# PoloWlg/Joint-Multimodal-Transformer-6th-ABAW

Hardware: AMD Instinct MI355X
Metric: train windows/sec + CCC parity, B=64 T=300 A/V fusion, 1/2/4/8 MI355X (higher is better)
Workload: dtype bf16; 1 GPU; configs[2]: FcLayer(1024,512) + Two_transformers(TRANSFORMER,FC,H=1,L=1,vision_in_ft=2048) + 2x CCCLoss + SGD-nesterov; global_batch=64, per_gpu_batch=64, seq_len=300, D_a=1024, D_v=2048, parallelism=dp1

## Files before the change

### include/jmt.h

```cpp
#ifndef JMT_H_
#define JMT_H_

#include <stddef.h>
#include <stdint.h>

#ifdef __cplusplus
extern "C" {
#endif

#define JMT_ABI_VERSION 7

enum { JMT_F32 = 0, JMT_BF16 = 1, JMT_F16 = 2 };
enum { JMT_OK = 0, JMT_ERR_ARG = -1, JMT_ERR_HIP = -2, JMT_ERR_UNSUPPORTED = -3 };

int jmt_abi_version(void);
const char* jmt_last_error(void);
int jmt_kernel_count(void);
long long jmt_bounds_violations(int reset);

typedef struct jmt_gemm_desc {
  int ab_dtype, c_dtype, aux_dtype;
  int M, N, K;
  const void* a[8];
  const void* b[8];
  void* c[8];
  int n_a, n_b, n_c;
  int a_mode, b_mode, c_mode;
  int a_kseg, b_kseg;
  int a_kmajor, b_kmajor;
  int64_t lda, ldb, ldc, ldaux;
  int batch0, batch1;
  int64_t sA0, sA1, sB0, sB1, sC0, sC1;
  float alpha, beta;
  const float* bias;
  int bias_mode;
  int relu;
  const void* aux;
  int splits;
  void* workspace;
  size_t ws_bytes;
  const float* bias_tab[8];
  int n_bias;
  float* dbias_tab[8];
  int n_dbias;
  int dbias_acc;
  float* dbias_ws;
  size_t dbias_ws_bytes;
} jmt_gemm_desc;

int jmt_gemm(const jmt_gemm_desc* desc, void* stream);
int jmt_gemm_cin(const jmt_gemm_desc* desc, const void* const* c_in, int n_c_in, int64_t ldcin,
                 void* stream);
int jmt_gemm_persist_cfg(const jmt_gemm_desc* desc);
size_t jmt_gemm_workspace_bytes(int M, int N, int batch, int splits);
int jmt_gemm_plan_splits(int ab_dtype, int M, int N, int K, int batch);
void jmt_gemm_set_debug(int flags);
int jmt_gemm_trace_read(uint64_t* host, int nblocks);

int jmt_gemm_grouped(const jmt_gemm_desc* descs, int n, void* workspace, size_t ws_bytes,
                     void* stream);
size_t jmt_gemm_grouped_workspace_bytes(const jmt_gemm_desc* descs, int n);
int jmt_gemm_grouped_plan(const jmt_gemm_desc* descs, int n, int* splits_out);

int jmt_gemm_group16(const jmt_gemm_desc* descs, int n, void* stream);
int jmt_gemm_group16_ok(const jmt_gemm_desc* descs, int n);
void jmt_gemm_group16_set_grid(int blocks);


int jmt_l2norm_fwd(int x_dt, int y_dt, int64_t rows, int D, const void* x, int64_t ldx, void* y,
                   int64_t ldy, float* inv_norm, float eps, void* stream);
int jmt_l2norm_bwd(int x_dt, int dy_dt, int dx_dt, int64_t rows, int D, const void* x,
                   int64_t ldx, const void* dy, int64_t lddy, const float* inv_norm, float eps,
                   void* dx, int64_t lddx, void* stream);

int jmt_layernorm_fwd(int dt_in, int dt_out, int64_t rows, int D, const void* x, int64_t ldx,
                      const void* r, int64_t ldr, const float* gamma, const float* beta, float eps,
                      void* y, int64_t ldy, float* mean, float* rstd, void* stream);
int jmt_layernorm_bwd_blocks(int64_t rows);
int jmt_layernorm_bwd(int dt_in, int dt_dy, int dt_dx, int64_t rows, int D, const void* x,
                      int64_t ldx, const void* r, int64_t ldr, const void* dy, int64_t lddy,
                      const float* mean, const float* rstd, const float* gamma, void* dx,
                      int64_t lddx, float* dgamma, float* dbeta, int beta_acc, float* partials,
                      void* stream);

int jmt_layernorm_bwd_dsum(int dt_in, int dt_dy, int dt_dx, int64_t rows, int D, const void* x,
                           int64_t ldx, const void* r, int64_t ldr, const void* dy, int64_t lddy,
                           const float* mean, const float* rstd, const float* gamma, void* dx,
                           int64_t lddx, float* dgamma, float* dbeta, float* dsum, int beta_acc,
                           float* partials, void* stream);

int jmt_layernorm_fwd_grouped(int dt_in, int dt_out, int G, int64_t rows, int D, const void* x,
                              int64_t ldx, int64_t sx, const void* r, int64_t ldr, int64_t sr,
                              const float* const* gamma, const float* const* beta, float eps,
                              void* y, int64_t ldy, int64_t sy, float* mean, float* rstd,
                              void* stream);
int jmt_layernorm_bwd_grouped(int dt_in, int dt_dy, int dt_dx, int G, int64_t rows, int D,
                              const void* x, int64_t ldx, int64_t sx, const void* r, int64_t ldr,
                              int64_t sr, const void* dy, int64_t lddy, int64_t sdy,
                              const float* mean, const float* rstd, const float* const* gamma,
                              void* dx, int64_t lddx, int64_t sdx, float* const* dgamma,
                              float* const* dbeta, float* const* dsum, int beta_acc,
                              float* partials, void* stream);
int jmt_layernorm_bwd_grouped_blocks(int64_t rows);

int jmt_softmax_fwd(int p_dt, int64_t rows, int n, const float* s, int64_t lds, float scale,
                    void* p, int64_t ldp, void* stream);
int jmt_softmax_bwd(int p_dt, int ds_dt, int64_t rows, int n, const void* p, int64_t ldp,
                    const float* dp, int64_t lddp, float scale, void* ds, int64_t ldds,
// ... 294 lines not shown
```

### joint-multimodal-transformer-6th-abaw_amd/csrc/gemm.hip

```cpp
#include "gemm_tile.h"

namespace jmt {

struct GemmWork {
  int m0, n0, b, b0, b1, split, kbeg, kend;
};

template <class C>
__device__ __forceinline__ GemmWork decode_work(const GemmParams& p, int w) {
  const int ntile = p.tiles_m * p.tiles_n;
  const int nb = p.batch0 * p.batch1;
  const bool global = p.splits > 1 && !(p.dbg & 16);
  if (global) {
    const int W = ntile * nb * p.splits;
    const int q = W / 8, rm = W % 8, x = w % 8;
    w = x * q + min(x, rm) + w / 8;
  }
  const int bid = w % ntile;
  const int rest = w / ntile;
  GemmWork r;
  r.b = rest % nb;
  r.split = rest / nb;
  int wg = bid;
  if (!global && ntile >= 16) {
// ... 515 lines not shown
      cfg = 44;
      splits = s;
      return;
    }
  }
  const TileModel* ms = dt == JMT_F32 ? kModels32 : kModels16;
  const int nm = dt == JMT_F32 ? 1 : 2;
  double best = 1e300;
  cfg = 1;
  splits = fixed_splits > 0 ? fixed_splits : 1;
  for (int i = 0; i < nm; ++i) {
    if (!tile_ok(ms[i], M, N)) continue;
    const long tiles = (long)((M + ms[i].bm - 1) / ms[i].bm) * ((N + ms[i].bn - 1) / ms[i].bn) *
                       batch;
    int s_lo = 1, s_hi = tiles <= 8 ? 256 : 32;
    if (fixed_splits > 0) s_lo = s_hi = fixed_splits;
    for (int s = s_lo; s <= s_hi; ++s) {
      if (fixed_splits <= 0 && s > 1 && K / s < 4 * bke) break;
      const double c = model_cost(ms[i], M, N, K, batch, s, bke);
      if (c < best * 0.999) { best = c; cfg = ms[i].id; splits = s; }
    }
  }
}

}

using namespace jmt;

static int g_gemm_dbg = 0;
static int g_gemm_cfg = 0;
extern "C" int jmt_gemm_trace_read(uint64_t* host, int nblocks) {
  if (nblocks > kTraceBlocks) nblocks = kTraceBlocks;
  if (hipDeviceSynchronize() != hipSuccess ||
      hipMemcpyFromSymbol(host, HIP_SYMBOL(g_gemm_trace), sizeof(uint64_t) * 4 * nblocks) !=
          hipSuccess)
    return -1;
  return nblocks;
}
extern "C" void jmt_gemm_set_debug(int flags) { g_gemm_dbg = flags & 0xff; g_gemm_cfg = flags >> 8; }

extern "C" int jmt_gemm_plan_splits(int ab_dtype, int M, int N, int K, int batch) {
  if (M <= 0 || N <= 0 || K <= 0) return 1;
  if (ab_dtype != JMT_F32 && ab_dtype != JMT_BF16 && ab_dtype != JMT_F16) return 1;
  int cfg, splits;
  plan(ab_dtype, M, N, K, batch < 1 ? 1 : batch, 0, cfg, splits);
  return splits;
}

extern "C" size_t jmt_gemm_workspace_bytes(int M, int N, int batch, int splits) {
  if (splits <= 1) return 0;
  return (size_t)splits * (size_t)batch * (size_t)M * (size_t)N * sizeof(float);
}

static int gemm_run(const jmt_gemm_desc* d, bool cin, const void* const* c_in, int n_c_in,
                    int64_t ldcin, void* stream, int* plan_out = nullptr) {
  JMT_CHECK_ARG(d != nullptr, "jmt_gemm: null descriptor");
  const int dt = d->ab_dtype;
  JMT_CHECK_ARG(dt == JMT_F32 || dt == JMT_BF16 || dt == JMT_F16, "jmt_gemm: bad ab_dtype %d", dt);
  JMT_CHECK_ARG(d->c_dtype == JMT_F32 || d->c_dtype == dt, "jmt_gemm: c_dtype must be f32 or ab");
  JMT_CHECK_ARG(d->M >= 0 && d->N >= 0 && d->K >= 0, "jmt_gemm: negative size");
  JMT_CHECK_ARG(d->aux == nullptr || d->aux_dtype == d->c_dtype,
                "jmt_gemm: aux (ReLU mask) must have the output dtype");
  if (d->M == 0 || d->N == 0) return JMT_OK;
  const int batch0 = d->batch0 < 1 ? 1 : d->batch0;
  const int batch1 = d->batch1 < 1 ? 1 : d->batch1;
  JMT_CHECK_ARG(batch0 * batch1 <= 65535, "jmt_gemm: batch too large");
  const int es = dtype_size(dt);
  const int V = 16 / es;
  const int BKE = 128 / es;
  JMT_CHECK_ARG(d->n_a >= 1 && d->n_a <= MAXP && d->n_b >= 1 && d->n_b <= MAXP &&
                    d->n_c >= 1 && d->n_c <= MAXP, "jmt_gemm: pointer table size");
  JMT_CHECK_ARG(d->lda % V == 0 && d->ldb % V == 0, "jmt_gemm: lda/ldb must be multiples of %d", V);
  JMT_CHECK_ARG((d->sA0 % V == 0) && (d->sA1 % V == 0) && (d->sB0 % V == 0) && (d->sB1 % V == 0),
                "jmt_gemm: batch strides must be multiples of %d elements", V);
  for (int i = 0; i < d->n_a; ++i)
    JMT_CHECK_ARG(((uintptr_t)d->a[i] & 15) == 0, "jmt_gemm: A[%d] not 16-B aligned", i);
  for (int i = 0; i < d->n_b; ++i)
    JMT_CHECK_ARG(((uintptr_t)d->b[i] & 15) == 0, "jmt_gemm: B[%d] not 16-B aligned", i);
  JMT_CHECK_ARG(d->a_mode >= 0 && d->a_mode <= 3 && d->b_mode >= 0 && d->b_mode <= 3 &&
                    d->c_mode >= 0 && d->c_mode <= 1, "jmt_gemm: bad operand mode");
  if (d->a_mode == 2) JMT_CHECK_ARG(d->a_kseg % BKE == 0 && d->a_kseg * d->n_a >= d->K,
                                    "jmt_gemm: A K-concat segment must be a multiple of %d", BKE);
  if (d->b_mode == 2) JMT_CHECK_ARG(d->b_kseg % BKE == 0 && d->b_kseg * d->n_b >= d->K,
                                    "jmt_gemm: B K-concat segment must be a multiple of %d", BKE);
  const int nseg_a = d->a_mode == 3 && d->a_kseg > 0 ? (d->K + d->a_kseg - 1) / d->a_kseg : 1;
  const int nseg_b = d->b_mode == 3 && d->b_kseg > 0 ? (d->K + d->b_kseg - 1) / d->b_kseg : 1;
  if (d->a_mode == 3) JMT_CHECK_ARG(d->a_kseg > 0 && d->a_kseg % BKE == 0 &&
                                        d->n_a >= batch0 * nseg_a && d->batch1 <= 1,
                                    "jmt_gemm: A per-batch K-concat needs kseg a multiple of %d, "
                                    "batch0 x ceil(K / kseg) pointers and batch1 = 1", BKE);
  if (d->b_mode == 3) JMT_CHECK_ARG(d->b_kseg > 0 && d->b_kseg % BKE == 0 &&
                                        d->n_b >= batch0 * nseg_b && d->batch1 <= 1,
                                    "jmt_gemm: B per-batch K-concat needs kseg a multiple of %d, "
                                    "batch0 x ceil(K / kseg) pointers and batch1 = 1", BKE);
  if (d->a_mode == 1) JMT_CHECK_ARG(d->n_a >= batch0, "jmt_gemm: A pointer table < batch0");
  if (d->b_mode == 1) JMT_CHECK_ARG(d->n_b >= batch0, "jmt_gemm: B pointer table < batch0");
  if (d->c_mode == 1) JMT_CHECK_ARG(d->n_c >= batch0, "jmt_gemm: C pointer table < batch0");

  GemmParams p;
  for (int i = 0; i < MAXP; ++i) {
    p.a_ptr[i] = i < d->n_a ? d->a[i] : nullptr;
    p.b_ptr[i] = i < d->n_b ? d->b[i] : nullptr;
    p.c_ptr[i] = i < d->n_c ? d->c[i] : nullptr;
  }
  JMT_CHECK_ARG(d->n_bias >= 0 && d->n_bias <= MAXP, "jmt_gemm: bias table size");
  if (d->n_bias > 0)
    JMT_CHECK_ARG(d->n_bias >= batch0 && d->bias_mode != 0, "jmt_gemm: bias table < batch0");
  p.bias = d->bias;
// ... 27 lines not shown
                  "dbias table of batch0 entries");
    bool any = false;
    for (int i = 0; i < batch0; ++i) any = any || d->dbias_tab[i] != nullptr;
    JMT_CHECK_ARG(any, "jmt_gemm: every dbias_tab entry is null");
  }
  {
    const int ces = dtype_size(d->c_dtype);
    bool cv4 = d->ldc % 4 == 0 && d->sC0 % 4 == 0 && d->sC1 % 4 == 0;
    for (int i = 0; i < d->n_c; ++i) cv4 = cv4 && (((uintptr_t)d->c[i] & (4 * ces - 1)) == 0);
    if (d->aux) cv4 = cv4 && (((uintptr_t)d->aux & (4 * ces - 1)) == 0) && d->ldaux % 4 == 0;
    p.c_vec4 = cv4 ? 1 : 0;
    bool cv8 = cv4 && d->ldc % 8 == 0 && d->sC0 % 8 == 0 && d->sC1 % 8 == 0;
    for (int i = 0; i < d->n_c; ++i) cv8 = cv8 && (((uintptr_t)d->c[i] & 15) == 0);
    p.c_vec8 = cv8 ? 1 : 0;
  }

  for (int i = 0; i < MAXP; ++i) p.cin_ptr[i] = p.c_ptr[i];
  p.ldcin = d->ldc;
  if (cin) {
    JMT_CHECK_ARG(d->beta != 0.f, "jmt_gemm_cin: beta == 0 reads no C operand");
    JMT_CHECK_ARG(c_in != nullptr && n_c_in >= (d->c_mode == 1 ? batch0 : 1) && n_c_in <= MAXP,
                  "jmt_gemm_cin: c_in table null or shorter than C's");
    for (int i = 0; i < n_c_in; ++i)
      JMT_CHECK_ARG(c_in[i] != nullptr && ((uintptr_t)c_in[i] & 15) == 0,
                    "jmt_gemm_cin: c_in[%d] null or not 16-B aligned", i);
    JMT_CHECK_ARG(ldcin >= d->N && ldcin % 8 == 0,
                  "jmt_gemm_cin: ldcin must be a multiple of 8 elements, at least N");
    if (d->c_dtype == JMT_F32 || dt == JMT_F32)
      return set_error(JMT_ERR_UNSUPPORTED, "jmt_gemm_cin: 16-bit C only");
    if (d->splits > 1)
      return set_error(JMT_ERR_UNSUPPORTED, "jmt_gemm_cin: split-K reduces into C itself");
    for (int i = 0; i < MAXP; ++i) p.cin_ptr[i] = i < n_c_in ? c_in[i] : nullptr;
    p.ldcin = ldcin;
  }

  int splits = d->splits < 1 ? 1 : d->splits;
  int kps = ((d->K + splits - 1) / splits + BKE - 1) / BKE * BKE;
  if (kps < BKE) kps = BKE;
  splits = (d->K + kps - 1) / kps;
  if (splits < 1) splits = 1;
  p.splits = splits;
  p.k_per_split = splits > 1 ? kps : (d->K > 0 ? d->K : 1);
  p.ws = (float*)d->workspace;
  if (splits > 1) {
    const size_t need = jmt_gemm_workspace_bytes(d->M, d->N, batch0 * batch1, splits);
    JMT_CHECK_ARG(d->workspace != nullptr && d->ws_bytes >= need,
                  "jmt_gemm: split-K needs %zu workspace bytes", need);
    if (d->n_dbias > 0) {
      const size_t dneed = (size_t)splits * batch0 * (size_t)d->M * sizeof(float);
      JMT_CHECK_ARG(d->dbias_ws != nullptr && d->dbias_ws_bytes >= dneed,
                    "jmt_gemm: split-K A row sums need %zu dbias_ws bytes", dneed);
    }
  }
  int cfg = g_gemm_cfg;
  {
    const int pc = persist_choice(d, p, splits, cfg);
    if (plan_out) {
      *plan_out = pc;
      return JMT_OK;
    }
    if (pc) {
      p.tiles_m = (d->M + 255) / 256;
      p.tiles_n = d->N / 256;
      const int W = p.tiles_m * p.tiles_n * batch0 * batch1;
      const int ncu = num_cus_persist();
      const int blocks = W < ncu ? W : ncu;
      launch_gemm_persist(p, dt, d->a_kmajor, d->b_kmajor, pc, blocks, as_stream(stream));
      JMT_LAUNCH_CHECK("jmt_gemm(persistent)");
      return JMT_OK;
    }
  }
  const bool pp_split = splits > 1 && pp_split_ok(dt, d->M, d->N, d->K, splits) &&
                        (cfg == 44 || (cfg == 0 && pp_split_env() &&
                                       pp_split_plan(dt, d->M, d->N, d->K, batch0 * batch1)));
  if (cfg == 44) cfg = 0;
  if (cfg == 40 || cfg == 43 || cfg == 45) cfg = 5;
  if (dt == JMT_F32 && cfg >= 10) cfg = 1;
  if (cfg == 32 && !d->a_kmajor) cfg = 5;
  if (!cfg) {
    int s_unused;
    plan(dt, d->M, d->N, d->K, batch0 * batch1, splits, cfg, s_unused);
    if (dt != JMT_F32 && (cfg == 1 || splits == 1)) {
      const int t = occupancy_override(d->a_kmajor, d->b_kmajor, d->M, d->N, d->K,
                                       batch0 * batch1, splits);
      if (t) cfg = t;
    }
  }
  if (d->n_dbias > 0 && cfg == 10) cfg = 5;
  hipStream_t st = as_stream(stream);
  if (pp_split) {
    p.tiles_m = d->M / 256;
    p.tiles_n = d->N / 256;
    const int W = p.tiles_m * p.tiles_n * batch0 * batch1 * splits;
    const int ncu = num_cus_persist();
    launch_gemm_pp_split(p, dt, d->a_kmajor, d->b_kmajor, d->n_dbias > 0, W < ncu ? W : ncu, st);
    JMT_LAUNCH_CHECK("jmt_gemm(split-K ping-pong)");
  } else {
    int bm, bn;
    cfg_tile(cfg, bm, bn);
    p.tiles_m = (d->M + bm - 1) / bm;
    p.tiles_n = (d->N + bn - 1) / bn;
    dim3 grid(p.tiles_m * p.tiles_n, batch0 * batch1, splits);
    if (dt == JMT_F32) launch_t<float>(p, d->a_kmajor, d->b_kmajor, cfg, grid, st);
    else if (dt == JMT_BF16) launch_t<__bf16>(p, d->a_kmajor, d->b_kmajor, cfg, grid, st);
    else launch_t<_Float16>(p, d->a_kmajor, d->b_kmajor, cfg, grid, st);
    JMT_LAUNCH_CHECK("jmt_gemm");
  }
  if (splits > 1) {
    const bool v4 = d->N % 4 == 0 && p.c_vec4;
    const int64_t total = (int64_t)d->M * d->N * batch0 * batch1 / (v4 ? 4 : 1);
    int blocks = (int)((total + 255) / 256);
    if (blocks > 8192) blocks = 8192;
#define JMT_SKR(O)                                                                          \
    if (v4) hipLaunchKernelGGL((splitk_reduce_kernel<O, true>), dim3(blocks), dim3(256), 0, st, p); \
    else hipLaunchKernelGGL((splitk_reduce_kernel<O, false>), dim3(blocks), dim3(256), 0, st, p);
    if (d->c_dtype == JMT_F32) { JMT_SKR(float) }
    else if (d->c_dtype == JMT_BF16) { JMT_SKR(__bf16) }
    else { JMT_SKR(_Float16) }
#undef JMT_SKR
    JMT_LAUNCH_CHECK("jmt_gemm(splitk_reduce)");
  }
  return JMT_OK;
}

extern "C" int jmt_gemm(const jmt_gemm_desc* d, void* stream) {
  return gemm_run(d, false, nullptr, 0, 0, stream);
}

extern "C" int jmt_gemm_cin(const jmt_gemm_desc* d, const void* const* c_in, int n_c_in,
                            int64_t ldcin, void* stream) {
  return gemm_run(d, true, c_in, n_c_in, ldcin, stream);
}

extern "C" int jmt_gemm_persist_cfg(const jmt_gemm_desc* d) {
  int pc = 0;
  return gemm_run(d, false, nullptr, 0, 0, nullptr, &pc) == JMT_OK ? pc : 0;
}

namespace {

constexpr double kKtUs = 2.5, kItemUs = 8.0, kSlabUs = 0.065;

struct GroupPlan {
  int splits[GRP_MAXPROB];
  int64_t ws_off[GRP_MAXPROB], rs_off[GRP_MAXPROB];
  int64_t ws_floats;
  int items;
  bool rs;
};

int norm_splits(int K, int s) {
  for (int it = 0; it < 8; ++it) {
    int kps = ((K + s - 1) / s + 63) / 64 * 64;
    if (kps < 64) kps = 64;
    const int s2 = (K + kps - 1) / kps;
    if (s2 == s) break;
    s = s2;
  }
  return s < 1 ? 1 : s;
}

int group_check_one(const jmt_gemm_desc* d, const jmt_gemm_desc* d0, int i, int& pool) {
#define JMT_GRP_UNSUP(cond, ...) \
  do { if (!(cond)) return set_error(JMT_ERR_UNSUPPORTED, __VA_ARGS__); } while (0)
  const int dt = d->ab_dtype;
  JMT_CHECK_ARG(dt == JMT_F32 || dt == JMT_BF16 || dt == JMT_F16,
                "jmt_gemm_grouped: problem %d: bad ab_dtype %d", i, dt);
  JMT_GRP_UNSUP(dt != JMT_F32, "jmt_gemm_grouped: problem %d: fp32 operands", i);
  JMT_GRP_UNSUP(d->c_dtype == JMT_F32, "jmt_gemm_grouped: problem %d: c_dtype must be fp32", i);
  JMT_GRP_UNSUP(dt == d0->ab_dtype && !d->a_kmajor == !d0->a_kmajor &&
                    !d->b_kmajor == !d0->b_kmajor,
                "jmt_gemm_grouped: problem %d: one operand dtype and layout per group", i);
  JMT_CHECK_ARG(d->M > 0 && d->N > 0 && d->K > 0, "jmt_gemm_grouped: problem %d: empty size", i);
  JMT_GRP_UNSUP(d->M % 256 == 0 && d->N % 256 == 0 && d->K % 64 == 0 && d->K >= 256,
                "jmt_gemm_grouped: problem %d: M and N must be multiples of 256, K of 64 (>= 256)",
                i);
  JMT_GRP_UNSUP(d->bias == nullptr && d->n_bias == 0 && !d->relu && d->aux == nullptr,
                "jmt_gemm_grouped: problem %d: bias, relu and aux are not supported", i);
  JMT_GRP_UNSUP(d->batch1 <= 1, "jmt_gemm_grouped: problem %d: batch1 must be 1", i);
  const int batch0 = d->batch0 < 1 ? 1 : d->batch0;
  JMT_CHECK_ARG(d->n_a >= 1 && d->n_a <= MAXP && d->n_b >= 1 && d->n_b <= MAXP && d->n_c >= 1 &&
                    d->n_c <= MAXP && d->n_dbias >= 0 && d->n_dbias <= MAXP,
                "jmt_gemm_grouped: problem %d: pointer table size", i);
  JMT_GRP_UNSUP((d->a_mode == 0 || d->a_mode == 1 || d->a_mode == 3) &&
                    (d->b_mode == 0 || d->b_mode == 1 || d->b_mode == 3) &&
                    (d->c_mode == 0 || d->c_mode == 1),
                "jmt_gemm_grouped: problem %d: operand modes 0, 1 and 3 only", i);
  JMT_CHECK_ARG(d->lda > 0 && d->ldb > 0 && d->ldc > 0 && d->lda < (1LL << 31) &&
                    d->ldb < (1LL << 31) && d->ldc < (1LL << 31) && d->lda % 8 == 0 &&
// ... 415 lines not shown
```

### joint-multimodal-transformer-6th-abaw_amd/jmt/_lib.py

```python
from __future__ import annotations

import ctypes as C
import os

_HERE = os.path.dirname(os.path.abspath(__file__))
LIB_PATH = os.environ.get("JMT_LIB") or os.path.join(_HERE, "libjmt_hip.so")

F32, BF16, F16 = 0, 1, 2
OK, ERR_ARG, ERR_HIP, ERR_UNSUPPORTED = 0, -1, -2, -3

c_i64 = C.c_int64
c_vp = C.c_void_p
c_int = C.c_int
c_f = C.c_float
c_fp = C.POINTER(C.c_float)


class GemmDesc(C.Structure):
    _fields_ = [
        ("ab_dtype", c_int), ("c_dtype", c_int), ("aux_dtype", c_int),
        ("M", c_int), ("N", c_int), ("K", c_int),
        ("a", c_vp * 8), ("b", c_vp * 8), ("c", c_vp * 8),
        ("n_a", c_int), ("n_b", c_int), ("n_c", c_int),
        ("a_mode", c_int), ("b_mode", c_int), ("c_mode", c_int),
        ("a_kseg", c_int), ("b_kseg", c_int),
        ("a_kmajor", c_int), ("b_kmajor", c_int),
        ("lda", c_i64), ("ldb", c_i64), ("ldc", c_i64), ("ldaux", c_i64),
        ("batch0", c_int), ("batch1", c_int),
        ("sA0", c_i64), ("sA1", c_i64), ("sB0", c_i64), ("sB1", c_i64),
        ("sC0", c_i64), ("sC1", c_i64),
        ("alpha", c_f), ("beta", c_f),
        ("bias", c_vp), ("bias_mode", c_int), ("relu", c_int),
        ("aux", c_vp),
        ("splits", c_int),
        ("workspace", c_vp), ("ws_bytes", C.c_size_t),
        ("bias_tab", c_vp * 8), ("n_bias", c_int),
        ("dbias_tab", c_vp * 8), ("n_dbias", c_int), ("dbias_acc", c_int),
        ("dbias_ws", c_vp), ("dbias_ws_bytes", C.c_size_t),
    ]


_PROTOS = {
    "jmt_abi_version": (c_int, []),
    "jmt_last_error": (C.c_char_p, []),
    "jmt_kernel_count": (c_int, []),
    "jmt_bounds_violations": (C.c_longlong, [c_int]),
    "jmt_gemm": (c_int, [C.POINTER(GemmDesc), c_vp]),
    "jmt_gemm_workspace_bytes": (C.c_size_t, [c_int, c_int, c_int, c_int]),
    "jmt_gemm_plan_splits": (c_int, [c_int, c_int, c_int, c_int, c_int]),
    "jmt_gemm_grouped": (c_int, [C.POINTER(GemmDesc), c_int, c_vp, C.c_size_t, c_vp]),
    "jmt_gemm_grouped_workspace_bytes": (C.c_size_t, [C.POINTER(GemmDesc), c_int]),
    "jmt_gemm_grouped_plan": (c_int, [C.POINTER(GemmDesc), c_int, C.POINTER(c_int)]),
    "jmt_gemm_group16": (c_int, [C.POINTER(GemmDesc), c_int, c_vp]),
    "jmt_gemm_group16_ok": (c_int, [C.POINTER(GemmDesc), c_int]),
    "jmt_gemm_group16_set_grid": (None, [c_int]),
    "jmt_gemm_persist_cfg": (c_int, [C.POINTER(GemmDesc)]),
    "jmt_gemm_cin": (c_int, [C.POINTER(GemmDesc), c_vp, c_int, c_i64, c_vp]),
    "jmt_gemm_set_debug": (None, [c_int]),
    "jmt_gemm_trace_read": (c_int, [c_vp, c_int]),
    "jmt_l2norm_fwd": (c_int, [c_int, c_int, c_i64, c_int, c_vp, c_i64, c_vp, c_i64, c_vp, c_f,
                               c_vp]),
    "jmt_l2norm_bwd": (c_int, [c_int, c_int, c_int, c_i64, c_int, c_vp, c_i64, c_vp, c_i64, c_vp,
                               c_f, c_vp, c_i64, c_vp]),
    "jmt_layernorm_fwd": (c_int, [c_int, c_int, c_i64, c_int, c_vp, c_i64, c_vp, c_i64, c_vp,
                                  c_vp, c_f, c_vp, c_i64, c_vp, c_vp, c_vp]),
    "jmt_layernorm_bwd_blocks": (c_int, [c_i64]),
    "jmt_layernorm_bwd": (c_int, [c_int, c_int, c_int, c_i64, c_int, c_vp, c_i64, c_vp, c_i64,
                                  c_vp, c_i64, c_vp, c_vp, c_vp, c_vp, c_i64, c_vp, c_vp, c_int,
                                  c_vp, c_vp]),
    "jmt_layernorm_bwd_dsum": (c_int, [c_int, c_int, c_int, c_i64, c_int, c_vp, c_i64, c_vp,
                                       c_i64, c_vp, c_i64, c_vp, c_vp, c_vp, c_vp, c_i64, c_vp,
                                       c_vp, c_vp, c_int, c_vp, c_vp]),
    "jmt_layernorm_fwd_grouped": (c_int, [c_int, c_int, c_int, c_i64, c_int, c_vp, c_i64, c_i64,
                                          c_vp, c_i64, c_i64, c_vp, c_vp, c_f, c_vp, c_i64, c_i64,
                                          c_vp, c_vp, c_vp]),
    "jmt_layernorm_bwd_grouped": (c_int, [c_int, c_int, c_int, c_int, c_i64, c_int, c_vp, c_i64,
                                          c_i64, c_vp, c_i64, c_i64, c_vp, c_i64, c_i64, c_vp,
                                          c_vp, c_vp, c_vp, c_i64, c_i64, c_vp, c_vp, c_vp, c_int,
                                          c_vp, c_vp]),
    "jmt_softmax_fwd": (c_int, [c_int, c_i64, c_int, c_vp, c_i64, c_f, c_vp, c_i64, c_vp]),
    "jmt_softmax_bwd": (c_int, [c_int, c_int, c_i64, c_int, c_vp, c_i64, c_vp, c_i64, c_f, c_vp,
                                c_i64, c_vp]),
    "jmt_attn_supported": (c_int, [c_int, c_int]),
    "jmt_attn_fwd": (c_int, [c_int, c_int, c_int, c_int, c_int, c_int, c_vp, c_i64, c_i64, c_vp,
                             c_i64, c_i64, c_vp, c_i64, c_i64, c_vp, c_i64, c_i64, c_f, c_vp,
                             c_vp]),
    "jmt_attn_set_fwd_rows": (c_int, [c_int]),
    "jmt_attn_bwd": (c_int, [c_int, c_int, c_int, c_int, c_int, c_int, c_vp, c_i64, c_i64, c_vp,
                             c_i64, c_i64, c_vp, c_i64, c_i64, c_vp, c_i64, c_i64, c_vp, c_i64,
                             c_i64, c_vp, c_vp, c_vp, c_i64, c_vp, c_i64, c_i64, c_f, c_vp]),
    "jmt_attn_short_supported": (c_int, [c_int, c_int, c_int, c_int]),
    "jmt_attn_short_fwd": (c_int, [c_int, c_int, c_int, c_int, c_int, c_int, c_vp, c_i64, c_i64,
                                   c_vp, c_i64, c_i64, c_vp, c_i64, c_i64, c_vp, c_i64, c_i64,
                                   c_f, c_vp, c_vp]),
    "jmt_attn_short_bwd": (c_int, [c_int, c_int, c_int, c_int, c_int, c_int, c_vp, c_i64, c_i64,
                                   c_vp, c_i64, c_i64, c_vp, c_i64, c_i64, c_vp, c_i64, c_i64,
                                   c_vp, c_i64, c_i64, c_vp, c_vp, c_i64, c_i64, c_vp, c_i64,
                                   c_i64, c_vp, c_i64, c_i64, c_f, c_vp]),
    "jmt_attn_dkdv": (c_int, [c_int, c_int, c_int, c_int, c_int, c_int, c_vp, c_vp, c_i64, c_vp,
                              c_i64, c_i64, c_vp, c_i64, c_i64, c_vp, c_i64, c_i64, c_vp, c_i64,
                              c_i64, c_vp, c_i64, c_i64, c_vp, c_i64, c_i64, c_vp]),
    "jmt_attn_fwd_sq": (c_int, [c_int, c_int, c_int, c_int, c_int, c_int, c_vp, c_i64, c_i64,
                                c_vp, c_i64, c_i64, c_vp, c_i64, c_i64, c_vp, c_i64, c_i64, c_f,
                                c_vp, c_int, C.POINTER(c_int), c_int, c_vp]),
    "jmt_attn_bwd_sq": (c_int, [c_int, c_int, c_int, c_int, c_int, c_int, c_vp, c_i64, c_i64,
                                c_vp, c_i64, c_i64, c_vp, c_i64, c_i64, c_vp, c_i64, c_i64, c_vp,
                                c_i64, c_i64, c_vp, c_vp, c_vp, c_i64, c_f, c_int,
                                C.POINTER(c_int), c_int, c_vp]),
    "jmt_attn_dkdv_sq": (c_int, [c_int, c_int, c_int, c_int, c_int, c_int, c_vp, c_vp, c_i64,
                                 c_vp, c_i64, c_i64, c_vp, c_i64, c_i64, c_vp, c_i64, c_i64, c_vp,
# ... 189 lines not shown
```

### joint-multimodal-transformer-6th-abaw_amd/jmt/ops.py

```python
from __future__ import annotations

import ctypes as C
import math
import os
from typing import Optional, Sequence

import torch

from . import _lib
from ._lib import BF16, F16, F32, GemmDesc

_DT = {torch.float32: F32, torch.bfloat16: BF16, torch.float16: F16}


def dt(t_or_dtype) -> int:
    d = t_or_dtype if isinstance(t_or_dtype, torch.dtype) else t_or_dtype.dtype
    try:
        return _DT[d]
    except KeyError:
        raise _lib.JMTError(f"unsupported dtype {d}") from None


def stream() -> int:
    return torch.cuda.current_stream().cuda_stream
# ... 41 lines not shown
    for i, p in enumerate(b):
        d.b[i] = p
    for i, p in enumerate(c):
        d.c[i] = p
    d.n_a, d.n_b, d.n_c = len(a), len(b), len(c)
    d.a_mode, d.b_mode, d.c_mode = a_mode, b_mode, c_mode
    d.a_kseg, d.b_kseg = a_kseg, b_kseg
    d.a_kmajor, d.b_kmajor = int(a_kmajor), int(b_kmajor)
    d.lda, d.ldb, d.ldc, d.ldaux = lda, ldb, ldc, ldaux
    d.batch0, d.batch1 = batch0, batch1
    d.sA0, d.sA1 = sA
    d.sB0, d.sB1 = sB
    d.sC0, d.sC1 = sC
    d.alpha, d.beta = alpha, beta
    d.bias = bias.data_ptr() if bias is not None else None
    d.bias_mode = bias_mode if (bias is not None or bias_tab) else 0
    if bias_tab:
        for i, t in enumerate(bias_tab):
            d.bias_tab[i] = t.data_ptr()
        d.n_bias = len(bias_tab)
    d.relu = int(relu)
    d.aux = aux.data_ptr() if aux is not None else None
    if dbias_tab:
        for i, t in enumerate(dbias_tab):
            d.dbias_tab[i] = t.data_ptr() if t is not None else None
        d.n_dbias = len(dbias_tab)
        d.dbias_acc = int(dbias_acc)
    fam = {(True, True): "gemm_NT", (True, False): "gemm_NN", (False, False): "gemm_TN",
           (False, True): "gemm_TT"}[(bool(a_kmajor), bool(b_kmajor))]
    info = {"family": fam, "ab_dtype": ab_dtype, "c_dtype": c_dtype,
            "a_kmajor": bool(a_kmajor), "b_kmajor": bool(b_kmajor), "M": M, "N": N,
            "K": K, "batch": batch0 * batch1, "beta": beta,
            "dbias": bool(dbias_tab),
            "flops": 2.0 * M * N * K * batch0 * batch1,
            "bytes": batch0 * batch1 * ((M + N) * K * (4 if ab_dtype == F32 else 2) +
                                        M * N * (4 if c_dtype == F32 else 2)),
            "inplace": any(p in list(c) for p in list(a) + list(b))}

    def single():
        sp = splits if splits is not None else auto_splits(M, N, K, batch0 * batch1, ab_dtype)
        d.splits = sp
        ws = None
        if sp > 1:
            nbytes = _lib.load().jmt_gemm_workspace_bytes(M, N, batch0 * batch1, sp)
            if dbias_tab:
                dbytes = sp * batch0 * M * 4
                ws = workspace(nbytes + dbytes, device)
                d.dbias_ws = ws.data_ptr() + nbytes
                d.dbias_ws_bytes = dbytes
            else:
                ws = workspace(nbytes, device)
            d.workspace = ws.data_ptr()
            d.ws_bytes = nbytes
        if c_in is not None:
            tab = (C.c_void_p * len(c_in))(*c_in)
            launch = lambda: _lib.check(_lib.load().jmt_gemm_cin(
                C.byref(d), tab, len(c_in), ldcin or ldc, stream()), "jmt_gemm_cin")
        else:
            launch = lambda: _lib.check(_lib.load().jmt_gemm(C.byref(d), stream()), "jmt_gemm")
        if _launch_hook is not None:
            _launch_hook(info, launch)
        else:
            launch()
        return ws

    if done is not None and splits is None and _wgrad_enqueue(
            _WgradEntry(d, info, single, done, tuple(keep), device), defer):
        return None
    if done is None and _g16["depth"] > 0:
        sp = splits if splits is not None else auto_splits(M, N, K, batch0 * batch1, ab_dtype)
        _g16["ents"].append((d, info, single, sp, c_in is not None, tuple(keep)))
        return None
    ws = single()
    if done is not None:
        done()
    return ws


_wgrad_group = {"on": os.environ.get("JMT_WGRAD_GROUP", "1") != "0"}
_wgrad_defer = {"mode": {"0": "off", "single": "single"}.get(
    os.environ.get("JMT_WGRAD_DEFER", "1"), "on")}


def wgrad_group_enabled() -> bool:
    return _wgrad_group["on"]


def wgrad_defer_mode() -> str:
    return _wgrad_defer["mode"] if _wgrad_group["on"] else "off"


class _WgradEntry:
    __slots__ = ("d", "info", "single", "done", "keep", "device", "stream")

    def __init__(self, d, info, single, done, keep, device, stream=None):
        self.d, self.info, self.single, self.done = d, info, single, done
        self.keep, self.device = keep, device
        self.stream = stream if stream is not None else torch.cuda.current_stream()


_wq = {"depth": 0, "scoped": [], "deferred": [], "task": None, "scope_defer": False}


def _wgrad_hold(kind: str, ents) -> bool:
    task = torch._C._current_graph_task_id()
    if task < 0:
# ... 767 lines not shown
```

Before: 18450 windows/s.

## Split GEMM rows: persistent full waves plus split-K tail for leftover tiles

Adds a row-split plan for single-entry 16-bit GEMMs on the persistent ping-pong kernel. When the tile count is not a multiple of the CU count, the leading rows that fill whole waves run on the persistent kernel, and the leftover rows run as a split-K launch so the tail wave uses more CUs. A fitted cost model decides when to split and how many splits to use, and the Python wrapper now queries the plan and allocates an fp32 workspace. This trades a partial final wave for an extra launch, a workspace allocation on every call, and a reduction pass over the tail rows.

```diff
diff --git a/include/jmt.h b/include/jmt.h
--- a/include/jmt.h
+++ b/include/jmt.h
@@ -54,6 +54,18 @@
 int jmt_gemm_persist_cfg(const jmt_gemm_desc* desc);
 size_t jmt_gemm_workspace_bytes(int M, int N, int batch, int splits);
 int jmt_gemm_plan_splits(int ab_dtype, int M, int N, int K, int batch);
+#define JMT_EPI_BIAS_COL 1
+#define JMT_EPI_BIAS_ROW 2
+#define JMT_EPI_RELU 4
+#define JMT_EPI_AUX 8
+#define JMT_EPI_BETA 16
+#define JMT_EPI_CIN 32
+#define JMT_EPI_ALPHA 64
+int jmt_gemm_plan_rowsplit(int ab_dtype, int a_kmajor, int b_kmajor, int M, int N, int K,
+                           int batch, int epilogue, int n_cu, int* m0, int* splits);
+int jmt_gemm_rowsplit(const jmt_gemm_desc* desc, int* m0, int* splits);
+size_t jmt_gemm_rowsplit_workspace_bytes(int M, int N, int m0, int splits);
+int jmt_gemm_set_rowsplit(int m0, int splits);
 void jmt_gemm_set_debug(int flags);
 int jmt_gemm_trace_read(uint64_t* host, int nblocks);
 
diff --git a/joint-multimodal-transformer-6th-abaw_amd/csrc/abi_check_rowsplit.cpp b/joint-multimodal-transformer-6th-abaw_amd/csrc/abi_check_rowsplit.cpp
--- /dev/null
+++ b/joint-multimodal-transformer-6th-abaw_amd/csrc/abi_check_rowsplit.cpp
@@ -0,0 +1,128 @@
+#include <stdint.h>
+#include <stdio.h>
+#include <string.h>
+
+#include "../../include/jmt.h"
+
+static int g_fail = 0;
+
+static void expect(const char* what, bool ok) {
+  if (!ok) {
+    fprintf(stderr, "FAIL %s\n", what);
+    ++g_fail;
+  }
+}
+
+static void expect_err(const char* what, int rc, const char* needle) {
+  const char* e = jmt_last_error();
+  const size_t n = e ? strnlen(e, 1024) : 0;
+  if (rc != JMT_ERR_ARG || n == 0 || n >= 512 || !strstr(e, needle)) {
+    fprintf(stderr, "FAIL %s: rc=%d err='%s'\n", what, rc, e ? e : "(null)");
+    ++g_fail;
+  }
+}
+
+static const uintptr_t kBase = 0x10000000;
+
+static jmt_gemm_desc prob(int M, int N, int K) {
+  jmt_gemm_desc d;
+  memset(&d, 0, sizeof(d));
+  d.ab_dtype = d.c_dtype = d.aux_dtype = JMT_BF16;
+  d.M = M; d.N = N; d.K = K;
+  d.a_kmajor = d.b_kmajor = 1;
+  d.lda = K; d.ldb = K; d.ldc = N;
+  d.batch0 = d.batch1 = 1;
+  d.alpha = 1.f;
+  d.n_a = d.n_b = d.n_c = 1;
+  d.a[0] = (const void*)(kBase + 0x100);
+  d.b[0] = (const void*)(kBase + 0x200);
+  d.c[0] = (void*)(kBase + 0x1000000);
+  d.splits = 1;
+  d.workspace = (void*)(kBase + 0x4000000);
+  d.ws_bytes = (size_t)1 << 30;
+  return d;
+}
+
+template <class F>
+static void forced_refused(const char* what, const char* needle, F mutate) {
+  jmt_gemm_desc d = prob(600, 512, 1024);
+  mutate(d);
+  expect_err(what, jmt_gemm(&d, nullptr), needle);
+}
+
+int main() {
+  if (jmt_abi_version() != JMT_ABI_VERSION) {
+    fprintf(stderr, "FAIL abi version\n");
+    return 1;
+  }
+  int m0 = -1, s = -1;
+  expect("plan, null outputs",
+         jmt_gemm_plan_rowsplit(JMT_BF16, 1, 1, 19200, 1024, 3072, 1, 0, 256, nullptr, nullptr) ==
+             jmt_gemm_plan_rowsplit(JMT_BF16, 1, 1, 19200, 1024, 3072, 1, 0, 256, &m0, &s));
+  expect("plan geometry", (s == 1 && m0 == 19200) || (m0 == 16384 && s >= 2 && 44 * s <= 256));
+  expect("plan fp32", !jmt_gemm_plan_rowsplit(JMT_F32, 1, 1, 19200, 1024, 3072, 1, 0, 256, &m0,
+                                              &s) && m0 == 19200 && s == 1);
+  expect("plan bad dtype", !jmt_gemm_plan_rowsplit(9, 1, 1, 19200, 1024, 3072, 1, 0, 256, &m0,
+                                                   &s));
+  expect("plan n_cu 0", !jmt_gemm_plan_rowsplit(JMT_BF16, 1, 1, 19200, 1024, 3072, 1, 0, 0, &m0,
+                                                &s));
+  expect("plan negative", !jmt_gemm_plan_rowsplit(JMT_BF16, 1, 1, -5, -1024, -64, 1, 0, 256,
+                                                  &m0, &s) && m0 == -5);
+  expect("plan huge", !jmt_gemm_plan_rowsplit(JMT_BF16, 1, 1, 2147483640, 2147483392, 2147483584,
+                                              1, 0, 1, &m0, &s) || s >= 2);
+  expect("workspace", jmt_gemm_rowsplit_workspace_bytes(19200, 1024, 16384, 5) ==
+                          (size_t)5 * 2816 * 1024 * 4 &&
+                          jmt_gemm_rowsplit_workspace_bytes(19200, 1024, 19200, 5) == 0 &&
+                          jmt_gemm_rowsplit_workspace_bytes(19200, 1024, 16384, 1) == 0 &&
+                          jmt_gemm_rowsplit_workspace_bytes(19200, 1024, 0, 4) == 0);
+  {
+    jmt_gemm_desc d = prob(19200, 1024, 3072);
+    const int y = jmt_gemm_rowsplit(&d, &m0, &s);
+    expect("query", (y == 1 && m0 == 16384 && s >= 2) || (y == 0 && m0 == 19200 && s == 1));
+    expect("query null", jmt_gemm_rowsplit(nullptr, &m0, &s) == 0 && s == 1);
+    expect("query null outputs", jmt_gemm_rowsplit(&d, nullptr, nullptr) == y);
+    d.lda = 3076;
+    expect("query refused desc", jmt_gemm_rowsplit(&d, &m0, &s) == 0 && m0 == 19200 && s == 1);
+  }
+  expect_err("m0 no multiple of 256", jmt_gemm_set_rowsplit(100, 2), "jmt_gemm_set_rowsplit");
+  expect_err("m0 negative", jmt_gemm_set_rowsplit(-256, 2), "jmt_gemm_set_rowsplit");
+  expect_err("m0 zero, splits set", jmt_gemm_set_rowsplit(0, 2), "jmt_gemm_set_rowsplit");
+  expect_err("splits 1", jmt_gemm_set_rowsplit(256, 1), "jmt_gemm_set_rowsplit");
+  expect("setter clear", jmt_gemm_set_rowsplit(0, 0) == JMT_OK);
+  jmt_gemm_set_debug(45 << 8);
+  expect("setter ok", jmt_gemm_set_rowsplit(256, 2) == JMT_OK);
+  static float biasv[4];
+  forced_refused("batch 3", "row split", [](jmt_gemm_desc& d) {
+    d.batch0 = 3; d.sA0 = 1 << 20; d.sC0 = 1 << 20;
+  });
+  forced_refused("fp32", "row split", [](jmt_gemm_desc& d) { d.ab_dtype = d.c_dtype = JMT_F32; });
+  forced_refused("MN-major A", "row split", [](jmt_gemm_desc& d) { d.a_kmajor = 0; d.lda = 600; });
+  forced_refused("relu", "row split", [](jmt_gemm_desc& d) { d.relu = 1; });
+  forced_refused("beta", "row split", [](jmt_gemm_desc& d) { d.beta = 1.f; });
+  forced_refused("aux", "row split", [](jmt_gemm_desc& d) { d.aux = (const void*)kBase; d.ldaux = 512; });
+  forced_refused("alpha", "row split", [](jmt_gemm_desc& d) { d.alpha = 2.f; });
+  forced_refused("bias per row", "row split", [](jmt_gemm_desc& d) {
+    d.bias = biasv; d.bias_mode = 2;
+  });
+  forced_refused("N not a tile", "row split", [](jmt_gemm_desc& d) { d.N = 384; d.ldc = 384; });
+  forced_refused("m0 >= M", "row split", [](jmt_gemm_desc& d) { d.M = 256; });
+  forced_refused("under 4 K-tiles per split", "row split", [](jmt_gemm_desc& d) {
+    d.K = 448; d.lda = d.ldb = 448;
+  });
+  forced_refused("leftover x splits over the CUs", "row split", [](jmt_gemm_desc& d) {
+    d.M = 256 * 70; d.N = 1024; d.ldc = 1024;
+  });
+  forced_refused("no workspace", "workspace", [](jmt_gemm_desc& d) { d.workspace = nullptr; });
+  forced_refused("short workspace", "workspace", [](jmt_gemm_desc& d) {
+    d.ws_bytes = (size_t)2 * 344 * 512 * 4 - 1;
+  });
+  jmt_gemm_set_debug(0);
+  forced_refused("not on the ping-pong kernel", "row split", [](jmt_gemm_desc&) {});
+  expect("setter clear", jmt_gemm_set_rowsplit(0, 0) == JMT_OK);
+  if (g_fail) {
+    fprintf(stderr, "abi_check_rowsplit: %d failure(s)\n", g_fail);
+    return 1;
+  }
+  printf("abi_check_rowsplit: ok\n");
+  return 0;
+}
diff --git a/joint-multimodal-transformer-6th-abaw_amd/csrc/gemm.hip b/joint-multimodal-transformer-6th-abaw_amd/csrc/gemm.hip
--- a/joint-multimodal-transformer-6th-abaw_amd/csrc/gemm.hip
+++ b/joint-multimodal-transformer-6th-abaw_amd/csrc/gemm.hip
@@ -591,8 +591,101 @@
   return (size_t)splits * (size_t)batch * (size_t)M * (size_t)N * sizeof(float);
 }
 
+constexpr double kRsA = 1.4312, kRsB = 15.72, kRsC = 7.31, kRsR = 0.4149, kRsPart = 0.68;
+
+static const char* rowsplit_refused(int dt, int ak, int M, int N, int K, int batch, int epi) {
+  if (batch != 1) return "a single entry only";
+  if (dt != JMT_BF16 && dt != JMT_F16) return "16-bit operands only";
+  if (!ak) return "K-major A only";
+  if (M <= 0 || N <= 0 || K < 128 || N % 256 || K % 64 || M % 8)
+    return "a shape the ping-pong kernel does not run";
+  if (epi & ~JMT_EPI_BIAS_COL) return "the plain or per-column bias epilogue only";
+  return nullptr;
+}
+
+static int rowsplit_norm(int K, int s) {
+  const int64_t kps = (((int64_t)K + s - 1) / s + 63) / 64 * 64;
+  return (int)((K + kps - 1) / kps);
+}
+
+static double rowsplit_cost(int M2, int N, int kt, int s) {
+  return kRsA * ((kt + s - 1) / s) + kRsC + kRsR * ((s + 0.5) * M2 * (double)N * 4.0 / 1e6);
+}
+
+static bool rowsplit_plan(int dt, int ak, int M, int N, int K, int batch, int epi, int n_cu,
+                          int& m0, int& splits) {
+  m0 = M;
+  splits = 1;
+  if (n_cu < 1 || rowsplit_refused(dt, ak, M, N, K, batch, epi)) return false;
+  const int C = N / 256, kt = K / 64;
+  const int64_t tiles = (((int64_t)M + 255) / 256) * C;
+  if (tiles <= n_cu || tiles % n_cu == 0) return false;
+  const int64_t k = tiles / n_cu;
+  const int64_t r0 = k * n_cu / C;
+  if (r0 < 1 || r0 * 256 >= M) return false;
+  const int M2 = M - (int)(r0 * 256);
+  const int64_t L = (((int64_t)M2 + 255) / 256) * C;
+  int best = 0;
+  double bc = 1e300;
+  for (int s = 2; L * s <= n_cu && kt / s >= 4; ++s) {
+    if (rowsplit_norm(K, s) != s) continue;
+    const double c = rowsplit_cost(M2, N, kt, s);
+    if (c < bc) { bc = c; best = s; }
+  }
+  if (!best) return false;
+  const double round = kRsA * kt + kRsB;
+  if (k * round + bc >= (double)((tiles + n_cu - 1) / n_cu) * round) return false;
+  m0 = (int)(r0 * 256);
+  splits = best;
+  return true;
+}
+
+static bool rowsplit_gains(int M, int N, int K, int n_cu, int m0, int s) {
+  const int kt = K / 64;
+  const int64_t t1 = (int64_t)(m0 / 256) * (N / 256);
+  const double k = (double)((t1 + n_cu - 1) / n_cu), round = kRsA * kt + kRsB;
+  return k * round + rowsplit_cost(M - m0, N, kt, s) < (k + kRsPart) * round;
+}
+
+static int g_rs_m0 = 0, g_rs_splits = 0;
+
+extern "C" int jmt_gemm_plan_rowsplit(int ab_dtype, int a_kmajor, int b_kmajor, int M, int N,
+                                      int K, int batch, int epilogue, int n_cu, int* m0,
+                                      int* splits) {
+  (void)b_kmajor;
+  int m = M, s = 1;
+  const bool y = rowsplit_plan(ab_dtype, a_kmajor, M, N, K, batch, epilogue, n_cu, m, s);
+  if (m0) *m0 = m;
+  if (splits) *splits = s;
+  return y ? 1 : 0;
+}
+
+extern "C" size_t jmt_gemm_rowsplit_workspace_bytes(int M, int N, int m0, int splits) {
+  if (splits <= 1 || m0 <= 0 || m0 >= M || N <= 0) return 0;
+  return (size_t)splits * (size_t)(M - m0) * (size_t)N * sizeof(float);
+}
+
+extern "C" int jmt_gemm_set_rowsplit(int m0, int splits) {
+  if (m0 == 0 && splits == 0) {
+    g_rs_m0 = g_rs_splits = 0;
+    return JMT_OK;
+  }
+  JMT_CHECK_ARG(m0 > 0 && m0 % 256 == 0, "jmt_gemm_set_rowsplit: m0 %d is no positive multiple "
+                "of 256", m0);
+  JMT_CHECK_ARG(splits >= 2, "jmt_gemm_set_rowsplit: splits %d < 2", splits);
+  g_rs_m0 = m0;
+  g_rs_splits = splits;
+  return JMT_OK;
+}
+
+static int rowsplit_env() {
+  const char* e = getenv("JMT_GEMM_ROWSPLIT");
+  return e ? atoi(e) : 1;
+}
+
 static int gemm_run(const jmt_gemm_desc* d, bool cin, const void* const* c_in, int n_c_in,
-                    int64_t ldcin, void* stream, int* plan_out = nullptr) {
+                    int64_t ldcin, void* stream, int* plan_out = nullptr, int* rs_out = nullptr,
+                    int part = 0) {
   JMT_CHECK_ARG(d != nullptr, "jmt_gemm: null descriptor");
   const int dt = d->ab_dtype;
   JMT_CHECK_ARG(dt == JMT_F32 || dt == JMT_BF16 || dt == JMT_F16, "jmt_gemm: bad ab_dtype %d", dt);
@@ -726,13 +819,76 @@
                     "jmt_gemm: split-K A row sums need %zu dbias_ws bytes", dneed);
     }
   }
-  int cfg = g_gemm_cfg;
+  int cfg = part == 1 ? 45 : part == 2 ? 44 : g_gemm_cfg;
   {
     const int pc = persist_choice(d, p, splits, cfg);
     if (plan_out) {
       *plan_out = pc;
       return JMT_OK;
     }
+    if (rs_out) {
+      rs_out[0] = d->M;
+      rs_out[1] = 1;
+    }
+    if (part == 0 && d->splits <= 1 && rowsplit_env() && (g_rs_m0 > 0 || pc == 45)) {
+      const int epi = (p.bias_mode == 1 ? JMT_EPI_BIAS_COL : 0) |
+                      (p.bias_mode == 2 ? JMT_EPI_BIAS_ROW : 0) | (d->relu ? JMT_EPI_RELU : 0) |
+                      (d->aux ? JMT_EPI_AUX : 0) | (d->beta != 0.f ? JMT_EPI_BETA : 0) |
+                      (cin ? JMT_EPI_CIN : 0) | (d->alpha != 1.f ? JMT_EPI_ALPHA : 0);
+      const int ncu = num_cus_persist();
+      int m0 = d->M, rs = 1;
+      bool take;
+      if (g_rs_m0 > 0) {
+        if (rs_out) {
+          if (g_rs_m0 < d->M) {
+            rs_out[0] = g_rs_m0;
+            rs_out[1] = g_rs_splits;
+          }
+          return JMT_OK;
+        }
+        const char* why = pc != 45 ? "the launch is not on the ping-pong kernel"
+                                   : rowsplit_refused(dt, d->a_kmajor, d->M, d->N, d->K,
+                                                      batch0 * batch1, epi);
+        JMT_CHECK_ARG(why == nullptr, "jmt_gemm: forced row split refused: %s", why);
+        m0 = g_rs_m0;
+        rs = g_rs_splits;
+        JMT_CHECK_ARG(m0 < d->M, "jmt_gemm: forced row split at m0 %d of M %d", m0, d->M);
+        const long L = (long)(((int64_t)d->M - m0 + 255) / 256) * (d->N / 256);
+        JMT_CHECK_ARG((d->K / 64) / rs >= 4 && rowsplit_norm(d->K, rs) == rs && L * rs <= ncu,
+                      "jmt_gemm: forced row split needs >= 4 whole K-tiles per split and "
+                      "leftover tiles x splits (%ld x %d) within %d CUs", L, rs, ncu);
+        const size_t need = jmt_gemm_rowsplit_workspace_bytes(d->M, d->N, m0, rs);
+        JMT_CHECK_ARG(d->workspace != nullptr && d->ws_bytes >= need,
+                      "jmt_gemm: forced row split needs %zu workspace bytes", need);
+        take = true;
+      } else {
+        take = rowsplit_plan(dt, d->a_kmajor, d->M, d->N, d->K, batch0 * batch1, epi, ncu, m0,
+                             rs) &&
+               (rowsplit_env() == 2 || rowsplit_gains(d->M, d->N, d->K, ncu, m0, rs));
+        if (take && rs_out) {
+          rs_out[0] = m0;
+          rs_out[1] = rs;
+          return JMT_OK;
+        }
+        take = take && d->workspace != nullptr &&
+               d->ws_bytes >= jmt_gemm_rowsplit_workspace_bytes(d->M, d->N, m0, rs);
+      }
+      if (take) {
+        jmt_gemm_desc d1 = *d, d2 = *d;
+        d1.M = m0;
+        d1.splits = 1;
+        d2.M = d->M - m0;
+        d2.splits = rs;
+        const int64_t aoff = (int64_t)m0 * d->lda * es;
+        const int64_t coff = (int64_t)m0 * d->ldc * dtype_size(d->c_dtype);
+        for (int i = 0; i < d->n_a; ++i) d2.a[i] = (const char*)d->a[i] + aoff;
+        for (int i = 0; i < d->n_c; ++i) d2.c[i] = (char*)d->c[i] + coff;
+        const int rc = gemm_run(&d1, false, nullptr, 0, 0, stream, nullptr, nullptr, 1);
+        if (rc != JMT_OK) return rc;
+        return gemm_run(&d2, false, nullptr, 0, 0, stream, nullptr, nullptr, 2);
+      }
+    }
+    if (rs_out) return JMT_OK;
     if (pc) {
       p.tiles_m = (d->M + 255) / 256;
       p.tiles_n = d->N / 256;
@@ -809,6 +965,17 @@
 extern "C" int jmt_gemm_persist_cfg(const jmt_gemm_desc* d) {
   int pc = 0;
   return gemm_run(d, false, nullptr, 0, 0, nullptr, &pc) == JMT_OK ? pc : 0;
+}
+
+extern "C" int jmt_gemm_rowsplit(const jmt_gemm_desc* d, int* m0, int* splits) {
+  int rs[2] = {d ? d->M : 0, 1};
+  if (gemm_run(d, false, nullptr, 0, 0, nullptr, nullptr, rs) != JMT_OK) {
+    rs[0] = d ? d->M : 0;
+    rs[1] = 1;
+  }
+  if (m0) *m0 = rs[0];
+  if (splits) *splits = rs[1];
+  return rs[1] > 1 ? 1 : 0;
 }
 
 namespace {
diff --git a/joint-multimodal-transformer-6th-abaw_amd/jmt/_lib.py b/joint-multimodal-transformer-6th-abaw_amd/jmt/_lib.py
--- a/joint-multimodal-transformer-6th-abaw_amd/jmt/_lib.py
+++ b/joint-multimodal-transformer-6th-abaw_amd/jmt/_lib.py
@@ -56,6 +56,11 @@
     "jmt_gemm_group16_set_grid": (None, [c_int]),
     "jmt_gemm_persist_cfg": (c_int, [C.POINTER(GemmDesc)]),
     "jmt_gemm_cin": (c_int, [C.POINTER(GemmDesc), c_vp, c_int, c_i64, c_vp]),
+    "jmt_gemm_plan_rowsplit": (c_int, [c_int, c_int, c_int, c_int, c_int, c_int, c_int, c_int,
+                                       c_int, C.POINTER(c_int), C.POINTER(c_int)]),
+    "jmt_gemm_rowsplit": (c_int, [C.POINTER(GemmDesc), C.POINTER(c_int), C.POINTER(c_int)]),
+    "jmt_gemm_rowsplit_workspace_bytes": (C.c_size_t, [c_int, c_int, c_int, c_int]),
+    "jmt_gemm_set_rowsplit": (c_int, [c_int, c_int]),
     "jmt_gemm_set_debug": (None, [c_int]),
     "jmt_gemm_trace_read": (c_int, [c_vp, c_int]),
     "jmt_l2norm_fwd": (c_int, [c_int, c_int, c_i64, c_int, c_vp, c_i64, c_vp, c_i64, c_vp, c_f,
diff --git a/joint-multimodal-transformer-6th-abaw_amd/jmt/ops.py b/joint-multimodal-transformer-6th-abaw_amd/jmt/ops.py
--- a/joint-multimodal-transformer-6th-abaw_amd/jmt/ops.py
+++ b/joint-multimodal-transformer-6th-abaw_amd/jmt/ops.py
@@ -117,6 +117,13 @@
                 ws = workspace(nbytes, device)
             d.workspace = ws.data_ptr()
             d.ws_bytes = nbytes
+        elif c_in is None and batch0 * batch1 == 1 and M > 256:
+            m0, rs = C.c_int(M), C.c_int(1)
+            if _lib.load().jmt_gemm_rowsplit(C.byref(d), C.byref(m0), C.byref(rs)):
+                nbytes = _lib.load().jmt_gemm_rowsplit_workspace_bytes(M, N, m0.value, rs.value)
+                ws = workspace(nbytes, device)
+                d.workspace = ws.data_ptr()
+                d.ws_bytes = nbytes
         if c_in is not None:
             tab = (C.c_void_p * len(c_in))(*c_in)
             launch = lambda: _lib.check(_lib.load().jmt_gemm_cin(
```

Result: no change. 18520 windows/s, median of 6 (+0.4%).
